# nloyfer/wgbs_tools

Measured on AMD Instinct MI355X. Metric: CpG-sites/sec segmented, higher is better.
Workload: dtype u8 counts -> u32 prefix sums -> f32/f64 log-likelihood (bit-exact with the reference)

## Files before the change

### wgbs_tools_amd/build.py

```python
import os
import os.path as op
import shutil
import subprocess
import sys

HERE = op.dirname(op.abspath(__file__))
CSRC = op.join(HERE, 'csrc')
ARCH = 'gfx950'
HIPFLAGS = ['--offload-arch=' + ARCH, '-O3', '-std=c++17', '-ffp-contract=off', '-fPIC', '-shared', '-pthread']

TARGETS = {
    'libwgbsseg.so': (['wgbsseg.hip'], ['owners.h', 'env.h', 'seg_kernels.h', 'block_plan.h', 'block_kernels.h', 'plain_dp.h', 'wave_prims.h', 'exact_log2.h', 'stitch.h', 'add_loci.h', 'table_io.h', 'pat_kernels.h', 'homog_kernels.h', 'bimodal_kernels.h', 'stats_kernels.h', 'pair_plan.h', 'pair_kernels.h', '../../include/wgbsseg.h']),
    'libwgbssynth.so': (['synth.hip'], []),
}


def source_hash():
    import hashlib
    srcs, hdrs = TARGETS['libwgbsseg.so']
    h = hashlib.sha256()
    for f in sorted(op.normpath(op.join(CSRC, x)) for x in srcs + hdrs):
        with open(f, 'rb') as fh:
            h.update(fh.read())
    return h.hexdigest()[:16]


def hipcc():
    for cand in (shutil.which('hipcc'), '/opt/rocm/bin/hipcc'):
        if cand and op.isfile(cand):
            return cand
    raise RuntimeError('hipcc not found: cannot build the gfx950 libraries')


PROGRAMS = {
    'segmentor': (['segmentor_main.cpp'], ['../../include/wgbsseg.h']),
# ... 40 lines not shown
```

### wgbs_tools_amd/csrc/seg_kernels.h

```cpp
#pragma once
#include <hip/hip_runtime.h>
#include <stddef.h>
#include <stdint.h>
#include "exact_log2.h"
#include "wave_prims.h"

#ifndef WG_CARRY_SHIFT
#define WG_CARRY_SHIFT  7
#endif
#define WG_SCAN_STAGED  512
#define WG_CARRY_G      (1 << WG_CARRY_SHIFT)
static_assert(WG_CARRY_SHIFT >= 4 && WG_CARRY_SHIFT <= 10, "k_scan: a lane vector is 16 sites, an iteration 1024");
#define WG_BLOCK        256
#define WG_WIN_TILE     1024
#define WG_PAIR_CAP     4096
#define WG_TRACE_WIN    32768
#define WG_NARROW_WMAX  60
#define WG_MEDIUM_WMAX  252
#define WG_MEDIUM_TS    16

__device__ const wg_log_tables g_wg_tables = WG_LOG_TABLES_INIT;

__device__ __forceinline__ void wg_fast_tables_to_lds(wg_fast_tables* ft, int tid, int nthreads)
{
    const double* f = reinterpret_cast<const double*>(g_wg_tables.f_tab);
    const double* d = reinterpret_cast<const double*>(g_wg_tables.d_tab);
    double* of = reinterpret_cast<double*>(ft->f_tab);
    double* od = reinterpret_cast<double*>(ft->d_fast);
// ... 636 lines not shown
            t[j] = in ? ((h >> 8) & 0xffu) : 0u;
            tot += m[j] | (t[j] << 16);
        }
        const uint32_t incl = wg_wave_incl_scan_dpp_u32(tot);
        const uint32_t excl = incl - tot;
        uint32_t em = run_m + (excl & 0xffffu), et = run_t + (excl >> 16);
#pragma unroll
        for (int j = 0; j < 4; j++) {
            const int x = sidx + j - hs;
            if (x >= x0 && x < cnt) dst[x - x0] = make_uint2(em, et);
            em += m[j]; et += t[j];
        }
        const uint32_t wt = (uint32_t)__builtin_amdgcn_readlane((int)incl, 63);
        run_m += wt & 0xffffu; run_t += wt >> 16;
    }
}

__device__ __forceinline__ int wg_group_start(const ChunkDesc& cd, int k)
{
    const int64_t a = (cd.start0 + k) & ~(int64_t)(WG_CARRY_G - 1);
    return a <= cd.start0 ? 0 : (int)(a - cd.start0);
}

template <int ROW>
__device__ __forceinline__ void wg_stage_local_rows(uint32_t* __restrict__ Et, const uint8_t* __restrict__ betas, int64_t pitch,
                                                    int s_first, int ns, const ChunkDesc& cd, int64_t n_total, int ka, int cnt,
                                                    int lane, int wv)
{
    constexpr bool WHOLE = ROW > 128;
    const int half = WHOLE ? 0 : lane >> 5, l5 = WHOLE ? lane : lane & 31;
    const int64_t abs0 = cd.start0 + ka;
    const int64_t al = abs0 & ~3LL;
    const int hs = (int)(abs0 - al);
    const int sidx = l5 * 4;
    const int64_t a = al + sidx;
    const int nsite = cnt - 1;
    for (int r0 = WHOLE ? wv : wv * 2; r0 < ns; r0 += (WHOLE ? 1 : 2) * (WG_BLOCK / 64)) {
        const int rr = r0 + half;
        const bool act = rr < ns;
        uint32_t w0 = 0, w1 = 0;
        if (act && sidx < nsite + hs) {
            const uint8_t* row = betas + (int64_t)(s_first + rr) * pitch;
            if (a + 4 <= n_total) {
                const uint2 v = *reinterpret_cast<const uint2*>(row + 2 * a);
                w0 = v.x; w1 = v.y;
            } else {
                for (int j = 0; j < 4; j++) if (a + j < n_total) {
                    const uint32_t h = (uint32_t)row[2 * (a + j)] | ((uint32_t)row[2 * (a + j) + 1] << 8);
                    if (j < 2) w0 |= h << (16 * j); else w1 |= h << (16 * (j - 2));
                }
            }
        }
        uint32_t mt[4];
        uint32_t tot = 0;
#pragma unroll
        for (int j = 0; j < 4; j++) {
            const uint32_t h = ((j < 2) ? w0 : w1) >> (16 * (j & 1));
            const int x = sidx + j - hs;
            const bool in = x >= 0 && x < nsite;
            mt[j] = in ? ((h & 0xffu) | ((h & 0xff00u) << 8)) : 0u;
            tot += mt[j];
        }
        const uint32_t incl = WHOLE ? wg_wave_incl_scan_dpp_u32(tot) : wg_half_incl_scan_dpp_u32(tot);
        uint32_t e = incl - tot;
        uint32_t* dst = Et + (size_t)rr * ROW;
#pragma unroll
        for (int j = 0; j < 4; j++) {
            const int x = sidx + j - hs;
            if (act && x >= 0 && x < cnt) dst[x] = e;
            e += mt[j];
        }
    }
}

template <int ROW>
__device__ __forceinline__ void wg_stage_local_rows_long(uint32_t* __restrict__ Et, const uint8_t* __restrict__ betas, int64_t pitch,
                                                     int s_first, int ns, const ChunkDesc& cd, int64_t n_total, int ka, int cnt,
                                                     int lane, int wv)
{
    const int64_t abs0 = cd.start0 + ka;
    const int64_t al = abs0 & ~3LL;
    const int hs = (int)(abs0 - al);
    const int nsite = cnt - 1;
    for (int rr = wv; rr < ns; rr += WG_BLOCK / 64) {
        const uint8_t* row = betas + (int64_t)(s_first + rr) * pitch;
        uint32_t* dst = Et + (size_t)rr * ROW;
        uint32_t run = 0;
        for (int p0 = 0; p0 < nsite + hs; p0 += 256) {
            const int sidx = p0 + lane * 4;
            const int64_t a = al + sidx;
            uint32_t w0 = 0, w1 = 0;
            if (sidx < nsite + hs) {
                if (a + 4 <= n_total) {
                    const uint2 v = *reinterpret_cast<const uint2*>(row + 2 * a);
// ... 7 lines not shown
            }
            uint32_t mt[4];
            uint32_t tot = 0;
#pragma unroll
            for (int j = 0; j < 4; j++) {
                const uint32_t h = ((j < 2) ? w0 : w1) >> (16 * (j & 1));
                const int x = sidx + j - hs;
                const bool in = x >= 0 && x < nsite;
                mt[j] = in ? ((h & 0xffu) | ((h & 0xff00u) << 8)) : 0u;
                tot += mt[j];
            }
            const uint32_t incl = wg_wave_incl_scan_dpp_u32(tot);
            uint32_t e = run + (incl - tot);
#pragma unroll
            for (int j = 0; j < 4; j++) {
                const int x = sidx + j - hs;
                if (x >= 0 && x < cnt) dst[x] = e;
                e += mt[j];
            }
            run += (uint32_t)__builtin_amdgcn_readlane((int)incl, 63);
        }
        if (lane == 0 && ((nsite + hs) & 255) == 0 && nsite < cnt) dst[nsite] = run;
    }
}

#define WG_WIDE_TK      128
#define WG_WIDE_TS      16

template <int TI, int FAST, int SPLIT, bool ONEG>
__global__ __launch_bounds__(WG_BLOCK) void k_cost(JobView J, StageView SV, CostArgs A, const TileDesc* __restrict__ tiles,
                                                   int64_t n_tiles, double* __restrict__ cost, int64_t n_tiles_padded)
{
    constexpr bool WIDE = SPLIT == 1;
    constexpr int WM = SPLIT == 2 ? WG_MEDIUM_WMAX : WG_NARROW_WMAX;
    static_assert(SPLIT != 2 || TI == WG_MEDIUM_TS, "a medium tile is one 16-site unit");
    constexpr int KS = WIDE ? WG_WIDE_TK + 1 : TI + WM + 1;
    constexpr int IS = WIDE ? WG_WIDE_TS + 1 : 0;
    constexpr bool KY = (FAST >= 2);
    constexpr bool DIVS = (FAST == 3);
    extern __shared__ __attribute__((aligned(16))) char smem[];
    static_assert(sizeof(wg_fast_tables) % 16 == 0 && sizeof(wg_d2) == 16, "the arrays behind the tables are 16-byte aligned");
    const size_t TB = KY ? (size_t)A.rows * (16 + 64) * sizeof(wg_d2) : sizeof(wg_fast_tables);
    wg_fast_tables* tb = reinterpret_cast<wg_fast_tables*>(smem);
    wg_d2* iyt = reinterpret_cast<wg_d2*>(smem);
    wg_d2* kyt = iyt + (size_t)A.rows * 16;
    const wg_d2* iy0 = iyt + (A.rows - 1) * 16;
    const wg_d2* ky0 = kyt + (A.rows - 1) * 64;
    uint2* Et = reinterpret_cast<uint2*>(smem + TB);
    uint2* St = Et + (size_t)A.NS * KS;
    uint32_t* Lt = reinterpret_cast<uint32_t*>(smem + TB);
    char* after = WIDE ? reinterpret_cast<char*>(St + (((size_t)A.NS * (KS + IS) + 1) & ~(size_t)1) - (size_t)A.NS * KS)
                       : reinterpret_cast<char*>(Lt + (((size_t)A.NS * KS + 3) & ~(size_t)3));
    struct Rec { int32_t offs, ea; int64_t sb; };
    Rec* rec = reinterpret_cast<Rec*>(after);
    int32_t* misc = reinterpret_cast<int32_t*>(rec + (TI + 1));
    uint8_t* cmap = reinterpret_cast<uint8_t*>(misc + 8);
    constexpr bool CMAP = !WIDE;

    const int tid = threadIdx.x, lane = tid & 63, wv = tid >> 6;
    const int nC = J.n_chunks;
    const int64_t G = A.xcd_group, jx = (int64_t)(blockIdx.x >> 3);
    const int64_t t = (jx / G) * (8 * G) + (int64_t)(blockIdx.x & 7) * G + (jx % G);
    if (t >= n_tiles) return;
    const TileDesc td = tiles[t];
    const int c = td.chunk;
    const ChunkDesc cd = J.chunks[c];
    const int ka = td.ka, nk = td.nk, kb = ka + nk;
    const int et_lo = WIDE ? td.et_lo : 0;
    const int et_hi = WIDE ? et_lo + WG_WIDE_TK : (1 << 30);
    const uint32_t cum0 = SV.cum0[(int64_t)SV.stage * nC + c];

    if (KY) wg_lookup_tables_to_lds(iyt, kyt, A.rows, A.tab, tid, WG_BLOCK);
    else wg_fast_tables_to_lds(tb, tid, WG_BLOCK);
    constexpr int PW = (TI + 63) / 64;
    if (wv < PW) {
        const int kl = wv * 64 + lane;
        const int k = ka + kl;
        const bool valid = kl < nk;
        int cnt = 0, is = 0, ie = -1;
        if (valid) {
            const int f = J.W16[cd.site_off + k];
            is = k > et_lo ? k : et_lo;
            ie = (k + f < et_hi ? k + f : et_hi) - 1;
            cnt = ie - is + 1;
            if (cnt < 0) cnt = 0;
// ... 68 lines not shown
            else while (hi - lo > 1) { const int mid = (lo + hi) >> 1; if (rec[mid].offs <= q) lo = mid; else hi = mid; }
            const Rec r = rec[lo];
            double acc = firstg ? 0.0 : accR[qi];
            auto term = [&](float nm, float nt) -> double {
                const float ll = FAST == 1 ? wg_sample_term(nm, nt, pc, pc2, tb, &g_wg_tables) : wg_sample_term_plain(nm, nt, pc, pc2, &g_wg_tables);
                return (double)ll;
            };
            if (WIDE) {
                const uint2* Ep = Et + (q + r.ea);
                const uint2* Sp = St + lo;
                auto one = [&](int sl) {
                    const uint2 pi = Ep[sl * KS];
                    const uint2 pk = Sp[sl * IS];
                    if (KY) acc += (double)wg_sample_term_pcpos_ks<DIVS>((float)(pi.x - pk.x), (float)(pi.y - pk.y), pc, pc2, iy0, ky0, &g_wg_tables);
                    else acc += term((float)(pi.x - pk.x), (float)(pi.y - pk.y));
                };
                int sl = 0;
                for (; sl + 4 <= ns; sl += 4) { one(sl); one(sl + 1); one(sl + 2); one(sl + 3); }
                for (; sl < ns; sl++) one(sl);
            } else {
                const uint32_t* Ep = Lt + (q + r.ea);
                const uint32_t* Sp = Lt + lo;
                auto one = [&](int sl) {
                    const uint32_t d = Ep[sl * KS] - Sp[sl * KS];
                    if (KY) acc += (double)wg_sample_term_pcpos_ks<DIVS>((float)(d & 0xffffu), (float)(d >> 16), pc, pc2, iy0, ky0, &g_wg_tables);
                    else acc += term((float)(d & 0xffffu), (float)(d >> 16));
                };
                int sl = 0;
                for (; sl + 4 <= ns; sl += 4) { one(sl); one(sl + 1); one(sl + 2); one(sl + 3); }
                for (; sl < ns; sl++) one(sl);
            }
            if (lastg) cb[r.sb + q] = acc;
            else accR[qi] = acc;
        }
    }
    if (A.finished != nullptr && tid == 0) __hip_atomic_fetch_add(A.finished, 1u, __ATOMIC_RELAXED, __HIP_MEMORY_SCOPE_AGENT);
}

#ifdef WGBSSEG_DP_TIMING
#define WG_DP_T(...) __VA_ARGS__
#else
#define WG_DP_T(...)
#endif
struct DpArgs { int32_t ringN; int32_t pad[3]; };

#define WG_DP_STATE_HDR 257

__device__ __forceinline__ double wg_ld_l2_f64(const double* p) { return __hip_atomic_load(p, __ATOMIC_RELAXED, __HIP_MEMORY_SCOPE_AGENT); }
__device__ __forceinline__ int32_t wg_ld_l2_i32(const int32_t* p) { return __hip_atomic_load(p, __ATOMIC_RELAXED, __HIP_MEMORY_SCOPE_AGENT); }

template <int NW, int BL>
struct DpRows {
    static constexpr int PER = (BL + NW - 1) / NW;
    double va[PER], vb[PER];
    uint32_t fmax;
    bool wideb;
};

struct DpMeta { uint32_t w, rel; };
// ... 993 lines not shown
```

### wgbs_tools_amd/csrc/wgbsseg.hip

```cpp
#include <hip/hip_runtime.h>
#include <algorithm>
#include <atomic>
#include <chrono>
#include <cstdarg>
#include <cstdio>
#include <cstdlib>
#include <cstring>
#include <deque>
#include <functional>
#include <initializer_list>
#include <memory>
#include <string>
#include <thread>
#include <vector>
#include <pthread.h>
#include <sched.h>
#include <sys/mman.h>
#if defined(__x86_64__) && !defined(__HIP_DEVICE_COMPILE__)
#include <emmintrin.h>
#endif

#include "../../include/wgbsseg.h"
#include "owners.h"
#include "seg_kernels.h"
// ... 82 lines not shown
    bool counted_live = false;
    double stage_gate_wide_evals = 100000.0, stage_min_evals_per_step = 21000.0;
    bool stage_gate_shared = false;
    int stage_gate = 768, last_stage_pct = -1, force_dp_mode = 0, force_ns = 0, force_ti = 0;
    double last_block_sums_ms = 0.0;
    int64_t table_blocks = 0;
    bool accumulate = false;
    std::vector<std::pair<int64_t, int64_t>> validated;
    DevBuf scan_pieces, divcheck, plan_sb;
    DevBuf bs_plan, bs_desc, bs_out;
    DevBuf mk_out, cv_in, cv_out;
    DevBuf st_ranges, st_parts;
    DevBuf ph_pairs, ph_edges, ph_out;
    std::vector<int32_t> h_stage_bounds;
    float divs_pc = -1.0f;
    bool divs_ok = false;
    int64_t last_dp_chunks = 0, last_dp_stride = 0;
    float divs_m_pc = -1.0f;
    bool divs_m_ok = false;
    bool divs_enabled = true, bs_general = false;
    int64_t scan_piece_sites = 4096;
    int medium_wmax = WG_MEDIUM_WMAX;
    bool dp_wlean = true, early = true, speculate = true, batch_marks = false;
    ~wgbsseg_ctx() { (void)hipSetDevice(device); (void)hipDeviceSynchronize(); }
};

namespace {

bool device_local_cpus(int device, NearCpus* out)
{
    out->valid = false;
    if (!env_flag("WGBSSEG_UPLOAD_PIN", true)) return false;
    char bus[64] = {0};
    if (hipDeviceGetPCIBusId(bus, (int)sizeof bus, device) != hipSuccess) { (void)hipGetLastError(); return false; }
    for (char* q = bus; *q; q++) if (*q >= 'A' && *q <= 'F') *q = (char)(*q - 'A' + 'a');
    char path[160];
    snprintf(path, sizeof path, "/sys/bus/pci/devices/%s/local_cpulist", bus);
    FILE* f = fopen(path, "r");
    if (!f) return false;
    char line[8192] = {0};
    const bool got = fgets(line, (int)sizeof line, f) != nullptr;
    fclose(f);
    if (!got) return false;
    const size_t bytes = CPU_ALLOC_SIZE(WG_MAX_CPUS);
    std::vector<unsigned long> allowed(bytes / sizeof(unsigned long), 0ul);
    out->bits.assign(bytes / sizeof(unsigned long), 0ul);
// ... 224 lines not shown
    HIP_TRY(c->evD.create(false));
    HIP_TRY(c->evS.create(false));
    for (auto& v : c->ev) HIP_TRY(v.create());
    const long long budget_mb = env_int("WGBSSEG_COST_BUDGET_MB", 0);
    c->cost_budget_bytes = (budget_mb > 0 ? budget_mb : 6144LL) << 20;
    c->force_stages = (int)env_int("WGBSSEG_FORCE_STAGES", 0);
    c->stage_gate = (int)env_int("WGBSSEG_STAGE_GATE", c->stage_gate, 0);
    c->stage_gate_shared = env_flag("WGBSSEG_STAGE_GATE_SHARED", false);
    c->stage_gate_wide_evals = env_double("WGBSSEG_STAGE_GATE_WIDE_EVALS", c->stage_gate_wide_evals);
    c->stage_min_evals_per_step = env_double("WGBSSEG_STAGE_MIN_EVALS", c->stage_min_evals_per_step);
    if (env_int("WGBSSEG_LAST_STAGE_PCT", -1) != -1) c->last_stage_pct = (int)env_int("WGBSSEG_LAST_STAGE_PCT", -1, 5, 800);
    c->force_dp_mode = (int)env_int("WGBSSEG_DP_MODE", 0, 0, 2);
    c->force_ns = (int)env_int("WGBSSEG_NS", 0);
    c->force_ti = (int)env_int("WGBSSEG_TI", 0);
    c->bs_general = env_flag("WGBSSEG_BLOCK_SUMS_GENERAL", false);
    c->divs_enabled = env_flag("WGBSSEG_DIV_SHORT", true);
    { const long long sp = env_int("WGBSSEG_SCAN_PIECE_SITES", 0); if (sp >= 1024) c->scan_piece_sites = sp & ~1023LL; }
    const int wm = (int)env_int("WGBSSEG_MEDIUM_WMAX", WG_MEDIUM_WMAX, 0, WG_MEDIUM_WMAX);
    c->medium_wmax = wm > WG_NARROW_WMAX ? wm : 0;
    c->dp_wlean = env_flag("WGBSSEG_DP_WLEAN", true);
    c->early = !env_flag("WGBSSEG_NO_EARLY", false);
    c->speculate = !env_flag("WGBSSEG_NO_SPECULATION", false);
    c->batch_marks = env_int("WGBSSEG_PROFILE", 0) >= 2;
    g_live_ctx[device & 63].fetch_add(1, std::memory_order_relaxed);
    c->counted_live = true;
    *out = c.release();
    return WGBSSEG_OK;
}
}
extern "C" {

int wgbsseg_create(int device, wgbsseg_ctx** out, char* err, size_t errlen) { return create_ctx(device, true, out, err, errlen); }

void wgbsseg_destroy(wgbsseg_ctx* c)
{
    if (!c) return;
    if (c->counted_live) g_live_ctx[c->device & 63].fetch_sub(1, std::memory_order_relaxed);
    const double t0 = wall_s();
    delete c;
    if (profiling()) fprintf(stderr, "[wgbsseg] destroy: %.1f ms\n", (wall_s() - t0) * 1e3);
}

static hipError_t own_rows(wgbsseg_ctx* c, int64_t n_samples, int64_t n_sites, int elem)
{
    const int64_t pitch = round_up(2 * elem * n_sites, 256) + 256;
    const hipError_t e = c->betas_own.ensure((size_t)pitch * (size_t)n_samples);
// ... 205 lines not shown
    return WGBSSEG_OK;
}

int launch_scan(wgbsseg_ctx* c, const Job& job, hipStream_t s, char* err, size_t errlen)
{
    const int64_t rows = (int64_t)job.v.n_chunks * job.v.n_samples;
    const int64_t blocks = (rows + (WG_BLOCK / 64) - 1) / (WG_BLOCK / 64);
    if (blocks > 0x7fffffff) { set_err(err, errlen, "too many (chunk, sample) rows"); return WGBSSEG_E_ARG; }
    hipLaunchKernelGGL(k_scan, dim3((unsigned)blocks), dim3(WG_BLOCK), 0, s, job.v, c->status.as<JobStatus>());
    HIP_TRY(hipGetLastError());
    return WGBSSEG_OK;
}

int report_bad_site(const wgbsseg_ctx* c, const JobStatus& st, char* err, size_t errlen)
{
    const long long s = (long long)(st.first_bad >> 40), site = (long long)(st.first_bad & ((1ULL << 40) - 1));
    uint8_t mc[2] = {0, 0};
    (void)hipMemcpy(mc, c->betas + s * c->pitch + 2 * site, 2, hipMemcpyDeviceToHost);
    set_err(err, errlen, "invalid data: sample %lld (0-based, argument order), site %lld (0-based): meth %d > cov %d",
            s, site + (long long)c->site_base, (int)mc[0], (int)mc[1]);
    return WGBSSEG_E_METH_GT_COV;
}

template <int TI, int FAST, int SPLIT>
hipError_t launch_cost(const JobView& v, const StageView& sv, const CostArgs& a, const TileDesc* td, int64_t tiles, double* cost, size_t lds, hipStream_t s)
{
    const int64_t padded = round_up(tiles, 8 * (int64_t)a.xcd_group);
    if (TI > 64 || a.NS >= v.n_samples)
        hipLaunchKernelGGL((k_cost<TI, FAST, SPLIT, true>), dim3((unsigned)padded), dim3(WG_BLOCK), lds, s, v, sv, a, td, tiles, cost, padded);
    else
        hipLaunchKernelGGL((k_cost<(TI > 64 ? 64 : TI), FAST, SPLIT, false>), dim3((unsigned)padded), dim3(WG_BLOCK), lds, s, v, sv, a, td, tiles, cost, padded);
    return hipGetLastError();
}

template <int FAST>
hipError_t launch_cost_fast(int cls, int TI, const JobView& v, const StageView& sv, const CostArgs& a, const TileDesc* td, int64_t tiles, double* cost, size_t lds, hipStream_t s)
{
    if (cls == 2) return launch_cost<WG_MEDIUM_TS, FAST, 2>(v, sv, a, td, tiles, cost, lds, s);
    if (cls == 1) return launch_cost<WG_WIDE_TS, FAST == 3 ? 2 : FAST, 1>(v, sv, a, td, tiles, cost, lds, s);
    if (TI == 128) return launch_cost<128, FAST, 0>(v, sv, a, td, tiles, cost, lds, s);
    if (TI == 64) return launch_cost<64, FAST, 0>(v, sv, a, td, tiles, cost, lds, s);
    if (TI == 32) return launch_cost<32, FAST, 0>(v, sv, a, td, tiles, cost, lds, s);
    return launch_cost<16, FAST, 0>(v, sv, a, td, tiles, cost, lds, s);
}
hipError_t launch_cost_class(int cls, int fast, int TI, const JobView& v, const StageView& sv, const CostArgs& a, const TileDesc* td, int64_t tiles, double* cost, size_t lds, hipStream_t s)
{
    return fast == 3 ? launch_cost_fast<3>(cls, TI, v, sv, a, td, tiles, cost, lds, s) : fast == 2 ? launch_cost_fast<2>(cls, TI, v, sv, a, td, tiles, cost, lds, s)
         : fast == 1 ? launch_cost_fast<1>(cls, TI, v, sv, a, td, tiles, cost, lds, s) : launch_cost_fast<0>(cls, TI, v, sv, a, td, tiles, cost, lds, s);
}

template <int FAST>
hipError_t set_cost_attrs()
{
    const void* fns[] = {reinterpret_cast<const void*>(&k_cost<128, FAST, 0, true>),
                         reinterpret_cast<const void*>(&k_cost<64, FAST, 0, true>), reinterpret_cast<const void*>(&k_cost<32, FAST, 0, true>),
                         reinterpret_cast<const void*>(&k_cost<16, FAST, 0, true>), reinterpret_cast<const void*>(&k_cost<WG_WIDE_TS, FAST == 3 ? 2 : FAST, 1, true>),
                         reinterpret_cast<const void*>(&k_cost<WG_MEDIUM_TS, FAST, 2, true>),
                         reinterpret_cast<const void*>(&k_cost<64, FAST, 0, false>), reinterpret_cast<const void*>(&k_cost<32, FAST, 0, false>),
                         reinterpret_cast<const void*>(&k_cost<16, FAST, 0, false>), reinterpret_cast<const void*>(&k_cost<WG_WIDE_TS, FAST == 3 ? 2 : FAST, 1, false>),
                         reinterpret_cast<const void*>(&k_cost<WG_MEDIUM_TS, FAST, 2, false>)};
    for (const void* f : fns) {
        const hipError_t e = hipFuncSetAttribute(f, hipFuncAttributeMaxDynamicSharedMemorySize, 160 * 1024);
        if (e != hipSuccess) return e;
    }
    return hipSuccess;
}
hipError_t set_kernel_attributes()
{
    hipError_t e = set_cost_attrs<0>();
    if (e == hipSuccess) e = set_cost_attrs<1>();
    if (e == hipSuccess) e = set_cost_attrs<2>();
    if (e == hipSuccess) e = set_cost_attrs<3>();
    const void* dps[] = {reinterpret_cast<const void*>(&k_dp<7, 64>), reinterpret_cast<const void*>(&k_dp<7, 64, true>),
                         reinterpret_cast<const void*>(&k_dp<7, 32>),
                         reinterpret_cast<const void*>(&k_dp<15, 32>)};
    for (const void* f : dps)
        if (e == hipSuccess) e = hipFuncSetAttribute(f, hipFuncAttributeMaxDynamicSharedMemorySize, 160 * 1024);
    return e;
}

void grow_events(std::vector<Event>& v, size_t n)
{
    while (v.size() < n) { v.emplace_back(); (void)v.back().create(); }
// ... 392 lines not shown
        if (hf[(size_t)i]) total += (int64_t)plain[(size_t)i].size();
        else { total += ooff[oi + 1] - ooff[oi]; oi++; }
    }
    borders_off[n_chunks] = total;
    int32_t* out = (*alloc)(total);
    if (!out) { set_err(err, errlen, "borders_out too small: need %lld ints", (long long)total); return WGBSSEG_E_CAPACITY; }
    oi = 0;
    for (int64_t i = 0; i < n_chunks; i++) {
        if (hf[(size_t)i]) memcpy(out + borders_off[i], plain[(size_t)i].data(), plain[(size_t)i].size() * 4);
        else { memcpy(out + borders_off[i], ob.data() + ooff[oi], (size_t)(ooff[oi + 1] - ooff[oi]) * 4); oi++; }
    }
    c->last_valid = false;
    return WGBSSEG_OK;
}

int Batch::tile_plan(char* err, size_t errlen)
{
    BatchPlan& p = plan;
    const float pc = P.pseudo_count;
    const int n_stages = p.n_stages;
    CostArgs base;
    memset(&base, 0, sizeof(base));
    base.pc = pc; base.pc2 = pc + pc;
    base.xcd_group = 64;
    base.cmap = 3;
    for (int k = 0; k < 3; k++) { ca[k] = base; ca[k].NS = p.NS[k]; ca[k].rows = p.rows[k]; }
    if (p.term_mode[0] == 2) {
        const bool same = c->lookup_pc == pc && c->lookup_rows[0] == p.rows[0] && c->lookup_rows[1] == p.rows[1] && c->lookup_rows[2] == p.rows[2] && c->lookup.p;
        if (!same) {
            static const wg_log_tables host_tabs = WG_LOG_TABLES_INIT;
            c->h_lookup.resize((size_t)(p.rows[0] + p.rows[1] + p.rows[2]) * 80);
            wg_d2* dst = c->h_lookup.data();
            for (int rows : p.rows) {
                for (int x = 0; x < rows * 16; x++) dst[x] = wg_ks_iy_entry(&host_tabs, rows, x);
                for (int x = 0; x < rows * 64; x++) dst[rows * 16 + x] = wg_ks_ky_entry(&host_tabs, rows, x);
                dst += (size_t)rows * 80;
            }
            HIP_TRY(c->lookup.ensure(c->h_lookup.size() * sizeof(wg_d2)));
            HIP_TRY(hipMemcpyAsync(c->lookup.p, c->h_lookup.data(), c->h_lookup.size() * sizeof(wg_d2), hipMemcpyHostToDevice, c->sA));
            c->lookup_pc = pc;
            for (int k = 0; k < 3; k++) c->lookup_rows[k] = p.rows[k];
        }
        const wg_d2* tab = c->lookup.as<wg_d2>();
        for (int k = 0; k < 3; k++) { ca[k].tab = tab; tab += (size_t)p.rows[k] * 80; }
    }
    const size_t sb_bytes = (size_t)(n_stages + 1) * 4;
    HIP_TRY(c->plan_sb.ensure(sb_bytes));
// ... 67 lines not shown
    HIP_TRY(c->tmp_borders.ensure((size_t)(job.sites_padded + nC) * 4));
    HIP_TRY(c->nb.ensure((size_t)nC * 4));
    out_head = (size_t)round_up((int64_t)(nC + 1) * 8, 16);
    c->out_par ^= 1;
    outb = &c->out_borders[c->out_par];
    HIP_TRY(outb->ensure(out_head + (size_t)(J + nC) * 4));
    for (auto* evs : {&c->ev_cost0, &c->ev_cost1, &c->ev_dp0, &c->ev_dp1, &c->ev_fork, &c->ev_join}) grow_events(*evs, n_stages);
    StageView sv;
    sv.cbase = c->plan_cbase.as<int64_t>(); sv.cum0 = c->plan_cum0.as<uint32_t>();
    sv.tbaseA = c->plan_tbase.as<int64_t>(); sv.tbaseB = sv.tbaseA + (size_t)n_stages * (nC + 1);
    sv.sb = c->plan_sb.as<int32_t>();
    DpArgs da = {p.ringN, {c->dp_wlean ? 0 : 1, 0, 0}};
#ifdef WGBSSEG_DP_TIMING
    da.pad[1] = (int)env_int("WGBSSEG_DP_DEBUG", 0);
#endif
    c->last_dp_chunks = nC; c->last_dp_stride = p.state_stride;
    const size_t lds_dp = 2 * 4096 * 8 + 128 * 8 + 64 * 12 + 16 + 1024 * 6;
    double* const dps = c->dpstate.as<double>();
    if (st.wide_units) HIP_TRY(hipStreamWaitEvent(c->sA, c->ev[EV_SCAN_END], 0));
    if (st.wide_units && p.gated) HIP_TRY(hipStreamWaitEvent(c->sA2, c->ev[EV_SCAN_END], 0));
    const bool divsA = c->divs_enabled && c->divs_ok && c->divs_pc == P.pseudo_count;
    const bool divsM = c->divs_enabled && c->divs_m_ok && c->divs_m_pc == P.pseudo_count;
    const int fast[3] = {p.term_mode[0] == 2 && divsA ? 3 : p.term_mode[0], p.term_mode[1], p.term_mode[2] == 2 && divsM ? 3 : p.term_mode[2]};
    for (int stg = 0; stg < n_stages; stg++) {
        const int64_t* const nt = &p.stage_tiles[3 * (size_t)stg];
        hipStream_t const sP = p.gated && (stg & 1) ? c->sA2 : c->sA;
        sv.stage = stg;
        double* cbuf = c->cost[stg % p.nbuf].as<double>();
        const bool side = nt[0] > 0 && (nt[1] > 0 || nt[2] > 0);
        hipStream_t const sSide = side ? (p.gated && (stg & 1) ? c->sA : c->sA2) : sP;
        if (stg >= p.nbuf) HIP_TRY(hipStreamWaitEvent(sP, c->ev_dp1[stg - p.nbuf], 0));
        if (p.gated) {
            const int64_t before = stg > 0 ? nt[-3] + nt[-2] + nt[-1] : 0;
            if (before > 0) {
                const double est_s = 10.0 * (double)p.stage_pairs[(size_t)stg - 1] * c->n_samples / 5e11;
                const long long max_ticks = (long long)(1e8 * std::min(2.0, std::max(0.005, est_s)));
                hipLaunchKernelGGL(k_stage_gate, dim3(1), dim3(64), 0, sP, (const uint32_t*)(c->stage_ctr.as<uint32_t>() + (stg - 1)),
                                   (uint32_t)std::max<int64_t>(1, before - c->stage_gate), max_ticks);
                HIP_TRY(hipGetLastError());
            }
            for (CostArgs& a : ca) a.finished = c->stage_ctr.as<uint32_t>() + stg;
        }
        HIP_TRY(hipEventRecord(c->ev_cost0[stg], sP));
        if (side) { HIP_TRY(hipEventRecord(c->ev_fork[stg], sP)); HIP_TRY(hipStreamWaitEvent(sSide, c->ev_fork[stg], 0)); }
        for (int k : {0, 2, 1})
            if (nt[k] > 0)
                HIP_TRY(launch_cost_class(k, fast[k], p.TI, v, sv, ca[k], c->tiles[k].as<TileDesc>() + tile0[k][(size_t)stg], nt[k], cbuf, p.lds[k], k == 0 ? sP : sSide));
        if (side) { HIP_TRY(hipEventRecord(c->ev_join[stg], sSide)); HIP_TRY(hipStreamWaitEvent(sP, c->ev_join[stg], 0)); }
        HIP_TRY(hipEventRecord(c->ev_cost1[stg], sP));
        HIP_TRY(hipStreamWaitEvent(c->sB, c->ev_cost1[stg], 0));
        HIP_TRY(hipEventRecord(c->ev_dp0[stg], c->sB));
        const bool dp16 = p.dp_mode == 0 && n_stages > 1 && stg + 1 < n_stages;
        if (dp16)                                  hipLaunchKernelGGL((k_dp16<3>), dim3((unsigned)nC), dim3(64 * 4), (size_t)(2 * 16 * 64 * 8 + WG_DP_META_RING * 6), c->sB, v, sv, cbuf, dps, p.state_stride);
        else if (p.dp_mode == 0 && p.all_narrow)   hipLaunchKernelGGL((k_dp<7, 64, true>), dim3((unsigned)nC), dim3(64 * 8), lds_dp, c->sB, v, sv, cbuf, da, dps, p.state_stride);
        else if (p.dp_mode == 0)                   hipLaunchKernelGGL((k_dp<7, 64>), dim3((unsigned)nC), dim3(64 * 8), lds_dp, c->sB, v, sv, cbuf, da, dps, p.state_stride);
        else if (p.dp_mode == 1)                   hipLaunchKernelGGL((k_dp<7, 32>), dim3((unsigned)nC), dim3(64 * 8), lds_dp, c->sB, v, sv, cbuf, da, dps, p.state_stride);
        else                                       hipLaunchKernelGGL((k_dp<15, 32>), dim3((unsigned)nC), dim3(64 * 16), lds_dp, c->sB, v, sv, cbuf, da, dps, p.state_stride);
        HIP_TRY(hipGetLastError());
        HIP_TRY(hipEventRecord(c->ev_dp1[stg], c->sB));
    }
    return WGBSSEG_OK;
}

int Batch::deliver(char* err, size_t errlen)
{
    int64_t* const d_boff = outb->as<int64_t>();
    int32_t* const d_bord = reinterpret_cast<int32_t*>(reinterpret_cast<char*>(outb->p) + out_head);
    HIP_TRY(hipEventRecord(c->ev[EV_TRACE0], c->sB));
    hipLaunchKernelGGL(k_trace, dim3((unsigned)nC), dim3(WG_BLOCK), 0, c->sB, job.v, c->tmp_borders.as<int32_t>(), c->nb.as<int32_t>());
    HIP_TRY(hipGetLastError());
// ... 1730 lines not shown
        set_err(err, errlen, "test_bimodal: the EM of block %llu (row of the blocks) did not settle within %d iterations", s->em_cap, WG_BIM_MAX_ITERS);
        return WGBSSEG_E_CAPACITY;
    }
    HIP_TRY(hipMemcpy(ll, b->res_f.p, (size_t)b->n_blocks * 24, hipMemcpyDeviceToHost));
    HIP_TRY(hipMemcpy(counts, b->res_i.p, (size_t)b->n_blocks * 24, hipMemcpyDeviceToHost));
    return WGBSSEG_OK;
}

double wgbsseg_bimodal_kernel_ms(wgbsseg_bimodal* b)
{
    return b ? b->feed.kernel_ms() : -1.0;
}

int wgbsseg_get_timings(const wgbsseg_ctx* c, wgbsseg_timings* out)
{
    if (!c || !out) return WGBSSEG_E_ARG;
    *out = c->tim;
    return WGBSSEG_OK;
}

int64_t wgbsseg_debug_fetch(wgbsseg_ctx* c, const char* what, void* out, int64_t cap_bytes)
{
    if (!c || !what || !out || !c->last_valid) return WGBSSEG_E_STATE;
    const void* src = nullptr;
    int64_t bytes = 0;
    if (!strcmp(what, "window")) { src = c->W16.p; bytes = c->last_sites * 2; }
    else if (!strcmp(what, "cum")) { src = c->cum32.p; bytes = c->last_sites * 4; }
    else if (!strcmp(what, "back")) { src = c->back16.p; bytes = c->last_sites * 2; }
    else if (!strcmp(what, "dpstate")) { src = c->dpstate.p; bytes = c->last_dp_chunks * c->last_dp_stride * 8; }
    else if (!strcmp(what, "cost")) { if (c->last_stages != 1) return WGBSSEG_E_STATE; src = c->cost[0].p; bytes = c->last_pairs * 8; }
    else return WGBSSEG_E_ARG;
    if (bytes > cap_bytes) return WGBSSEG_E_CAPACITY;
    if (hipSetDevice(c->device) != hipSuccess) return WGBSSEG_E_HIP;
    if (hipMemcpy(out, src, (size_t)bytes, hipMemcpyDeviceToHost) != hipSuccess) return WGBSSEG_E_HIP;
    return bytes;
}

int wgbsseg_debug_sample_terms(wgbsseg_ctx* c, const float* nmeth, const float* ntotal, int64_t count, float pseudo_count, float* out)
{
    char* err = nullptr; size_t errlen = 0;
    if (!c || !nmeth || !ntotal || !out || count < 1) return WGBSSEG_E_ARG;
    HIP_TRY(hipSetDevice(c->device));
    HIP_TRY(c->dbg_a.ensure((size_t)count * 4)); HIP_TRY(c->dbg_b.ensure((size_t)count * 4)); HIP_TRY(c->dbg_c.ensure((size_t)count * 4));
    HIP_TRY(hipMemcpyAsync(c->dbg_a.p, nmeth, (size_t)count * 4, hipMemcpyHostToDevice, c->sA));
    HIP_TRY(hipMemcpyAsync(c->dbg_b.p, ntotal, (size_t)count * 4, hipMemcpyHostToDevice, c->sA));
    const unsigned blocks = (unsigned)std::min<int64_t>((count + 255) / 256, 8192);
// ... 84 lines not shown
```

Baseline: 1.142 billion.

## Pair two narrow cost tiles per workgroup and prefetch the next tile's rows

Adds a k_cost_pair kernel in which each workgroup scores two consecutive narrow cost tiles (TI 64 or 128) from the same XCD group. While the first tile's term evaluation proceeds, the window, cum and first beta row words of the second tile are fetched into registers, to hide global load latency and amortise the LDS table staging across two tiles. It is enabled by default for ungated TI=64 narrow runs and selected through an env knob, with the row load and scan logic factored into shared helpers. The cost is higher register pressure from the prefetched fronts and half as many workgroups in flight.

Result: faster. 1.158 billion, median of 4 (+1.3%).

```diff
diff --git a/wgbs_tools_amd/build.py b/wgbs_tools_amd/build.py
--- a/wgbs_tools_amd/build.py
+++ b/wgbs_tools_amd/build.py
@@ -10,7 +10,7 @@
 HIPFLAGS = ['--offload-arch=' + ARCH, '-O3', '-std=c++17', '-ffp-contract=off', '-fPIC', '-shared', '-pthread']
 
 TARGETS = {
-    'libwgbsseg.so': (['wgbsseg.hip'], ['owners.h', 'env.h', 'seg_kernels.h', 'block_plan.h', 'block_kernels.h', 'plain_dp.h', 'wave_prims.h', 'exact_log2.h', 'stitch.h', 'add_loci.h', 'table_io.h', 'pat_kernels.h', 'homog_kernels.h', 'bimodal_kernels.h', 'stats_kernels.h', 'pair_plan.h', 'pair_kernels.h', '../../include/wgbsseg.h']),
+    'libwgbsseg.so': (['wgbsseg.hip'], ['owners.h', 'env.h', 'seg_kernels.h', 'cost_map.h', 'block_plan.h', 'block_kernels.h', 'plain_dp.h', 'wave_prims.h', 'exact_log2.h', 'stitch.h', 'add_loci.h', 'table_io.h', 'pat_kernels.h', 'homog_kernels.h', 'bimodal_kernels.h', 'stats_kernels.h', 'pair_plan.h', 'pair_kernels.h', '../../include/wgbsseg.h']),
     'libwgbssynth.so': (['synth.hip'], []),
 }
 
diff --git a/wgbs_tools_amd/csrc/cost_map.h b/wgbs_tools_amd/csrc/cost_map.h
--- /dev/null
+++ b/wgbs_tools_amd/csrc/cost_map.h
@@ -0,0 +1,15 @@
+#pragma once
+#include <stdint.h>
+#include "exact_log2.h"
+
+WG_HD int64_t wg_cost_tile(int64_t wg, int h, int per, int64_t G)
+{
+    const int64_t j = (wg >> 3) * per + h;
+    return (j / G) * (8 * G) + (wg & 7) * G + (j % G);
+}
+
+WG_HD int64_t wg_cost_grid(int64_t n_tiles, int per, int64_t G)
+{
+    const int64_t padded = (n_tiles + 8 * G - 1) / (8 * G) * (8 * G);
+    return ((padded + per - 1) / per + 7) / 8 * 8;
+}
diff --git a/wgbs_tools_amd/csrc/seg_kernels.h b/wgbs_tools_amd/csrc/seg_kernels.h
--- a/wgbs_tools_amd/csrc/seg_kernels.h
+++ b/wgbs_tools_amd/csrc/seg_kernels.h
@@ -4,6 +4,7 @@
 #include <stdint.h>
 #include "exact_log2.h"
 #include "wave_prims.h"
+#include "cost_map.h"
 
 #ifndef WG_CARRY_SHIFT
 #define WG_CARRY_SHIFT  7
@@ -686,6 +687,44 @@
     return a <= cd.start0 ? 0 : (int)(a - cd.start0);
 }
 
+__device__ __forceinline__ uint2 wg_local_row_words(const uint8_t* __restrict__ row, int64_t a, int64_t n_total, bool want)
+{
+    uint32_t w0 = 0, w1 = 0;
+    if (want) {
+        if (a + 4 <= n_total) {
+            const uint2 v = *reinterpret_cast<const uint2*>(row + 2 * a);
+            w0 = v.x; w1 = v.y;
+        } else {
+            for (int j = 0; j < 4; j++) if (a + j < n_total) {
+                const uint32_t h = (uint32_t)row[2 * (a + j)] | ((uint32_t)row[2 * (a + j) + 1] << 8);
+                if (j < 2) w0 |= h << (16 * j); else w1 |= h << (16 * (j - 2));
+            }
+        }
+    }
+    return make_uint2(w0, w1);
+}
+template <bool WHOLE>
+__device__ __forceinline__ void wg_local_row_scan(uint32_t* __restrict__ dst, const uint2 w, bool act, int sidx, int hs, int nsite, int cnt)
+{
+    uint32_t mt[4];
+    uint32_t tot = 0;
+#pragma unroll
+    for (int j = 0; j < 4; j++) {
+        const uint32_t h = ((j < 2) ? w.x : w.y) >> (16 * (j & 1));
+        const int x = sidx + j - hs;
+        const bool in = x >= 0 && x < nsite;
+        mt[j] = in ? ((h & 0xffu) | ((h & 0xff00u) << 8)) : 0u;
+        tot += mt[j];
+    }
+    const uint32_t incl = WHOLE ? wg_wave_incl_scan_dpp_u32(tot) : wg_half_incl_scan_dpp_u32(tot);
+    uint32_t e = incl - tot;
+#pragma unroll
+    for (int j = 0; j < 4; j++) {
+        const int x = sidx + j - hs;
+        if (act && x >= 0 && x < cnt) dst[x] = e;
+        e += mt[j];
+    }
+}
 template <int ROW>
 __device__ __forceinline__ void wg_stage_local_rows(uint32_t* __restrict__ Et, const uint8_t* __restrict__ betas, int64_t pitch,
                                                     int s_first, int ns, const ChunkDesc& cd, int64_t n_total, int ka, int cnt,
@@ -702,38 +741,8 @@
     for (int r0 = WHOLE ? wv : wv * 2; r0 < ns; r0 += (WHOLE ? 1 : 2) * (WG_BLOCK / 64)) {
         const int rr = r0 + half;
         const bool act = rr < ns;
-        uint32_t w0 = 0, w1 = 0;
-        if (act && sidx < nsite + hs) {
-            const uint8_t* row = betas + (int64_t)(s_first + rr) * pitch;
-            if (a + 4 <= n_total) {
-                const uint2 v = *reinterpret_cast<const uint2*>(row + 2 * a);
-                w0 = v.x; w1 = v.y;
-            } else {
-                for (int j = 0; j < 4; j++) if (a + j < n_total) {
-                    const uint32_t h = (uint32_t)row[2 * (a + j)] | ((uint32_t)row[2 * (a + j) + 1] << 8);
-                    if (j < 2) w0 |= h << (16 * j); else w1 |= h << (16 * (j - 2));
-                }
-            }
-        }
-        uint32_t mt[4];
-        uint32_t tot = 0;
-#pragma unroll
-        for (int j = 0; j < 4; j++) {
-            const uint32_t h = ((j < 2) ? w0 : w1) >> (16 * (j & 1));
-            const int x = sidx + j - hs;
-            const bool in = x >= 0 && x < nsite;
-            mt[j] = in ? ((h & 0xffu) | ((h & 0xff00u) << 8)) : 0u;
-            tot += mt[j];
-        }
-        const uint32_t incl = WHOLE ? wg_wave_incl_scan_dpp_u32(tot) : wg_half_incl_scan_dpp_u32(tot);
-        uint32_t e = incl - tot;
-        uint32_t* dst = Et + (size_t)rr * ROW;
-#pragma unroll
-        for (int j = 0; j < 4; j++) {
-            const int x = sidx + j - hs;
-            if (act && x >= 0 && x < cnt) dst[x] = e;
-            e += mt[j];
-        }
+        const uint2 w = wg_local_row_words(betas + (int64_t)(s_first + rr) * pitch, a, n_total, act && sidx < nsite + hs);
+        wg_local_row_scan<WHOLE>(Et + (size_t)rr * ROW, w, act, sidx, hs, nsite, cnt);
     }
 }
 
@@ -787,6 +796,14 @@
         }
         if (lane == 0 && ((nsite + hs) & 255) == 0 && nsite < cnt) dst[nsite] = run;
     }
+}
+
+template <int FAST>
+__device__ __forceinline__ double wg_packed_term(uint32_t d, float pc, float pc2, const wg_fast_tables* tb, const wg_d2* iy0, const wg_d2* ky0)
+{
+    const float nm = (float)(d & 0xffffu), nt = (float)(d >> 16);
+    if (FAST >= 2) return (double)wg_sample_term_pcpos_ks<FAST == 3>(nm, nt, pc, pc2, iy0, ky0, &g_wg_tables);
+    return (double)(FAST == 1 ? wg_sample_term(nm, nt, pc, pc2, tb, &g_wg_tables) : wg_sample_term_plain(nm, nt, pc, pc2, &g_wg_tables));
 }
 
 #define WG_WIDE_TK      128
@@ -824,8 +841,7 @@
 
     const int tid = threadIdx.x, lane = tid & 63, wv = tid >> 6;
     const int nC = J.n_chunks;
-    const int64_t G = A.xcd_group, jx = (int64_t)(blockIdx.x >> 3);
-    const int64_t t = (jx / G) * (8 * G) + (int64_t)(blockIdx.x & 7) * G + (jx % G);
+    const int64_t t = wg_cost_tile((int64_t)blockIdx.x, 0, 1, A.xcd_group);
     if (t >= n_tiles) return;
     const TileDesc td = tiles[t];
     const int c = td.chunk;
@@ -940,9 +956,7 @@
                 const uint32_t* Ep = Lt + (q + r.ea);
                 const uint32_t* Sp = Lt + lo;
                 auto one = [&](int sl) {
-                    const uint32_t d = Ep[sl * KS] - Sp[sl * KS];
-                    if (KY) acc += (double)wg_sample_term_pcpos_ks<DIVS>((float)(d & 0xffffu), (float)(d >> 16), pc, pc2, iy0, ky0, &g_wg_tables);
-                    else acc += term((float)(d & 0xffffu), (float)(d >> 16));
+                    acc += wg_packed_term<FAST>(Ep[sl * KS] - Sp[sl * KS], pc, pc2, tb, iy0, ky0);
                 };
                 int sl = 0;
                 for (; sl + 4 <= ns; sl += 4) { one(sl); one(sl + 1); one(sl + 2); one(sl + 3); }
@@ -953,6 +967,157 @@
         }
     }
     if (A.finished != nullptr && tid == 0) __hip_atomic_fetch_add(A.finished, 1u, __ATOMIC_RELAXED, __HIP_MEMORY_SCOPE_AGENT);
+}
+
+template <int TI, int FAST>
+__global__ __launch_bounds__(WG_BLOCK) void k_cost_pair(JobView J, StageView SV, CostArgs A, const TileDesc* __restrict__ tiles, int64_t n_tiles,
+                                                        double* __restrict__ cost)
+{
+    static_assert(TI == 64 || TI == 128, "paired tiles: the 64- and 128-start narrow tiles");
+    constexpr int WM = WG_NARROW_WMAX, KS = TI + WM + 1;
+    constexpr bool KY = (FAST >= 2), WHOLE = KS > 128;
+    constexpr int PW = (TI + 63) / 64;
+    constexpr int RPP = (WHOLE ? 1 : 2) * (WG_BLOCK / 64);
+    constexpr int NPRE = 4;
+    extern __shared__ __attribute__((aligned(16))) char smem[];
+    const size_t TB = KY ? (size_t)A.rows * (16 + 64) * sizeof(wg_d2) : sizeof(wg_fast_tables);
+    wg_fast_tables* tb = reinterpret_cast<wg_fast_tables*>(smem);
+    wg_d2* iyt = reinterpret_cast<wg_d2*>(smem);
+    wg_d2* kyt = iyt + (size_t)A.rows * 16;
+    const wg_d2* iy0 = iyt + (A.rows - 1) * 16;
+    const wg_d2* ky0 = kyt + (A.rows - 1) * 64;
+    uint32_t* Lt = reinterpret_cast<uint32_t*>(smem + TB);
+    struct Rec { int32_t offs, ea; int64_t sb; };
+    Rec* rec = reinterpret_cast<Rec*>(Lt + (((size_t)A.NS * KS + 3) & ~(size_t)3));
+    int32_t* misc = reinterpret_cast<int32_t*>(rec + (TI + 1));
+    uint8_t* cmap = reinterpret_cast<uint8_t*>(misc + 8);
+
+    const int tid = threadIdx.x, lane = tid & 63, wv = tid >> 6;
+    const int nC = J.n_chunks, ns = J.n_samples;
+    const int64_t t0 = wg_cost_tile((int64_t)blockIdx.x, 0, 2, A.xcd_group);
+    if (t0 >= n_tiles) return;
+    const int64_t t1 = wg_cost_tile((int64_t)blockIdx.x, 1, 2, A.xcd_group);
+    const int np = t1 < n_tiles ? 2 : 1;
+
+    if (KY) wg_lookup_tables_to_lds(iyt, kyt, A.rows, A.tab, tid, WG_BLOCK);
+    else wg_fast_tables_to_lds(tb, tid, WG_BLOCK);
+
+    const int half = WHOLE ? 0 : lane >> 5, sidx = (WHOLE ? lane : lane & 31) * 4;
+    struct Desc {
+        int32_t ka, nk;
+        uint32_t cum0;
+        int64_t start0, site_off;
+        int64_t cbase;
+    };
+    auto describe = [&](int64_t t) {
+        const TileDesc td = tiles[t];
+        const ChunkDesc* cd = J.chunks + td.chunk;
+        Desc D;
+        D.ka = td.ka; D.nk = td.nk; D.start0 = cd->start0; D.site_off = cd->site_off;
+        D.cum0 = SV.cum0[(int64_t)SV.stage * nC + td.chunk];
+        D.cbase = SV.cbase[(int64_t)SV.stage * nC + td.chunk];
+        return D;
+    };
+    struct Front {
+        int32_t f;
+        uint32_t cum;
+        uint2 w[NPRE];
+    };
+    auto fetch = [&](const Desc& D, Front& F) {
+        const int kl = wv * 64 + lane;
+        const bool valid = wv < PW && kl < D.nk;
+        F.f = valid ? (int)J.W16[D.site_off + D.ka + kl] : 0;
+        F.cum = valid ? J.cum32[D.site_off + D.ka + kl] : 0u;
+        const int64_t abs0 = D.start0 + D.ka, al = abs0 & ~3LL;
+        const bool inrow = sidx < D.nk + WM + (int)(abs0 - al);
+#pragma unroll
+        for (int p = 0; p < NPRE; p++) {
+            const int rr = (WHOLE ? wv : wv * 2) + p * RPP + half;
+            F.w[p] = wg_local_row_words(J.betas + (int64_t)rr * J.pitch, al + sidx, J.n_total, rr < ns && inrow);
+        }
+    };
+
+    const Desc D0 = describe(t0), D1 = describe(np > 1 ? t1 : t0);
+    const float pc = A.pc, pc2 = A.pc2;
+    auto score = [&](const Desc& D, const Front& F, bool more, const Desc& Dn, Front& N) {
+        const int ka = D.ka, nk = D.nk;
+        if (wv < PW) {
+            const int kl = wv * 64 + lane, k = ka + kl;
+            const bool valid = kl < nk;
+            const int cnt = F.f;
+            const uint32_t incl = wg_wave_incl_scan_dpp_u32((uint32_t)cnt);
+            if (kl < TI) {
+                const int32_t o = (int32_t)(incl - (uint32_t)cnt);
+                const int is = valid ? k : 0;
+                Rec r;
+                r.offs = o;
+                r.ea = is - o + 1 - ka;
+                r.sb = (valid ? (int64_t)(F.cum - D.cum0) - k : 0) + (is - o);
+                rec[kl] = r;
+            }
+            const uint32_t imax = wg_wave_max_u32(cnt > 0 ? (uint32_t)(k + cnt - 1) : 0u);
+            if (lane == 0) misc[2 * wv + 1] = (int32_t)imax;
+            if (lane == 63) misc[4 + wv] = (int32_t)incl;
+        }
+        __syncthreads();
+        const int imax = PW > 1 ? (misc[1] > misc[3] ? misc[1] : misc[3]) : misc[1];
+        const int Q = PW > 1 ? misc[4] + misc[5] : misc[4];
+        if (Q > 0) {
+            if (PW > 1) {
+                if (wv == 1 && lane < TI - 64) {
+                    const int q0 = misc[4];
+                    Rec& r = rec[64 + lane];
+                    r.offs += q0; r.sb -= q0; r.ea -= q0;
+                }
+                __syncthreads();
+            }
+            if (tid == 0) rec[nk].offs = Q;
+            if (tid < nk) {
+                const int o0 = rec[tid].offs, o1 = tid + 1 < nk ? rec[tid + 1].offs : Q;
+                const int sh = A.cmap;
+                for (int g = (o0 + (1 << sh) - 1) >> sh; (g << sh) < o1; g++) cmap[g] = (uint8_t)tid;
+            }
+            const int Ecnt = imax + 2 - ka, nsite = Ecnt - 1;
+            const int64_t abs0 = D.start0 + ka, al = abs0 & ~3LL;
+            const int hs = (int)(abs0 - al);
+#pragma unroll
+            for (int p = 0; p < NPRE; p++) {
+                const int r0 = (WHOLE ? wv : wv * 2) + p * RPP, rr = r0 + half;
+                if (r0 < ns) wg_local_row_scan<WHOLE>(Lt + (size_t)rr * KS, F.w[p], rr < ns, sidx, hs, nsite, Ecnt);
+            }
+            for (int r0 = (WHOLE ? wv : wv * 2) + NPRE * RPP; r0 < ns; r0 += RPP) {
+                const int rr = r0 + half;
+                const uint2 w = wg_local_row_words(J.betas + (int64_t)rr * J.pitch, al + sidx, J.n_total, rr < ns && sidx < nsite + hs);
+                wg_local_row_scan<WHOLE>(Lt + (size_t)rr * KS, w, rr < ns, sidx, hs, nsite, Ecnt);
+            }
+        }
+        if (more) fetch(Dn, N);
+        if (Q > 0) {
+            __syncthreads();
+            double* cb = cost + D.cbase;
+            for (int q = tid; q < Q; q += WG_BLOCK) {
+                int lo = (int)cmap[q >> A.cmap];
+                if (A.cmap) while (rec[lo + 1].offs <= q) lo++;
+                const Rec r = rec[lo];
+                double acc = 0.0;
+                const uint32_t* Ep = Lt + (q + r.ea);
+                const uint32_t* Sp = Lt + lo;
+                auto one = [&](int sl) { acc += wg_packed_term<FAST>(Ep[sl * KS] - Sp[sl * KS], pc, pc2, tb, iy0, ky0); };
+                int sl = 0;
+                for (; sl + 4 <= ns; sl += 4) { one(sl); one(sl + 1); one(sl + 2); one(sl + 3); }
+                for (; sl < ns; sl++) one(sl);
+                cb[r.sb + q] = acc;
+            }
+        }
+    };
+    Front F0, F1;
+    fetch(D0, F0);
+    score(D0, F0, np > 1, D1, F1);
+    if (np > 1) {
+        __syncthreads();
+        score(D1, F1, false, D1, F0);
+    }
+    if (A.finished != nullptr && tid == 0) __hip_atomic_fetch_add(A.finished, (uint32_t)np, __ATOMIC_RELAXED, __HIP_MEMORY_SCOPE_AGENT);
 }
 
 #ifdef WGBSSEG_DP_TIMING
diff --git a/wgbs_tools_amd/csrc/wgbsseg.hip b/wgbs_tools_amd/csrc/wgbsseg.hip
--- a/wgbs_tools_amd/csrc/wgbsseg.hip
+++ b/wgbs_tools_amd/csrc/wgbsseg.hip
@@ -128,6 +128,8 @@
     int64_t scan_piece_sites = 4096;
     int medium_wmax = WG_MEDIUM_WMAX;
     bool dp_wlean = true, early = true, speculate = true, batch_marks = false;
+    int cost_pair = 1;
+    int32_t last_cost_forms[2] = {0, 0};
     ~wgbsseg_ctx() { (void)hipSetDevice(device); (void)hipDeviceSynchronize(); }
 };
 
@@ -398,6 +400,7 @@
     c->early = !env_flag("WGBSSEG_NO_EARLY", false);
     c->speculate = !env_flag("WGBSSEG_NO_SPECULATION", false);
     c->batch_marks = env_int("WGBSSEG_PROFILE", 0) >= 2;
+    c->cost_pair = (int)env_int("WGBSSEG_COST_PAIR", c->cost_pair, 0, 2);
     g_live_ctx[device & 63].fetch_add(1, std::memory_order_relaxed);
     c->counted_live = true;
     *out = c.release();
@@ -649,10 +652,19 @@
     return WGBSSEG_E_METH_GT_COV;
 }
 
+constexpr int WG_XCD_GROUP = 64;
+static_assert(WG_XCD_GROUP % 2 == 0, "paired tiles: both slots of a workgroup in one XCD group");
+
 template <int TI, int FAST, int SPLIT>
-hipError_t launch_cost(const JobView& v, const StageView& sv, const CostArgs& a, const TileDesc* td, int64_t tiles, double* cost, size_t lds, hipStream_t s)
-{
-    const int64_t padded = round_up(tiles, 8 * (int64_t)a.xcd_group);
+hipError_t launch_cost(const JobView& v, const StageView& sv, const CostArgs& a, const TileDesc* td, int64_t tiles, double* cost, size_t lds, hipStream_t s, bool pair)
+{
+    const int64_t padded = wg_cost_grid(tiles, 1, a.xcd_group);
+    if constexpr (SPLIT == 0 && (TI == 64 || TI == 128)) {
+        if (pair && a.NS >= v.n_samples && a.xcd_group % 2 == 0) {
+            hipLaunchKernelGGL((k_cost_pair<TI, FAST>), dim3((unsigned)wg_cost_grid(tiles, 2, a.xcd_group)), dim3(WG_BLOCK), lds, s, v, sv, a, td, tiles, cost);
+            return hipGetLastError();
+        }
+    }
     if (TI > 64 || a.NS >= v.n_samples)
         hipLaunchKernelGGL((k_cost<TI, FAST, SPLIT, true>), dim3((unsigned)padded), dim3(WG_BLOCK), lds, s, v, sv, a, td, tiles, cost, padded);
     else
@@ -661,19 +673,19 @@
 }
 
 template <int FAST>
-hipError_t launch_cost_fast(int cls, int TI, const JobView& v, const StageView& sv, const CostArgs& a, const TileDesc* td, int64_t tiles, double* cost, size_t lds, hipStream_t s)
-{
-    if (cls == 2) return launch_cost<WG_MEDIUM_TS, FAST, 2>(v, sv, a, td, tiles, cost, lds, s);
-    if (cls == 1) return launch_cost<WG_WIDE_TS, FAST == 3 ? 2 : FAST, 1>(v, sv, a, td, tiles, cost, lds, s);
-    if (TI == 128) return launch_cost<128, FAST, 0>(v, sv, a, td, tiles, cost, lds, s);
-    if (TI == 64) return launch_cost<64, FAST, 0>(v, sv, a, td, tiles, cost, lds, s);
-    if (TI == 32) return launch_cost<32, FAST, 0>(v, sv, a, td, tiles, cost, lds, s);
-    return launch_cost<16, FAST, 0>(v, sv, a, td, tiles, cost, lds, s);
-}
-hipError_t launch_cost_class(int cls, int fast, int TI, const JobView& v, const StageView& sv, const CostArgs& a, const TileDesc* td, int64_t tiles, double* cost, size_t lds, hipStream_t s)
-{
-    return fast == 3 ? launch_cost_fast<3>(cls, TI, v, sv, a, td, tiles, cost, lds, s) : fast == 2 ? launch_cost_fast<2>(cls, TI, v, sv, a, td, tiles, cost, lds, s)
-         : fast == 1 ? launch_cost_fast<1>(cls, TI, v, sv, a, td, tiles, cost, lds, s) : launch_cost_fast<0>(cls, TI, v, sv, a, td, tiles, cost, lds, s);
+hipError_t launch_cost_fast(int cls, int TI, const JobView& v, const StageView& sv, const CostArgs& a, const TileDesc* td, int64_t tiles, double* cost, size_t lds, hipStream_t s, bool pair)
+{
+    if (cls == 2) return launch_cost<WG_MEDIUM_TS, FAST, 2>(v, sv, a, td, tiles, cost, lds, s, false);
+    if (cls == 1) return launch_cost<WG_WIDE_TS, FAST == 3 ? 2 : FAST, 1>(v, sv, a, td, tiles, cost, lds, s, false);
+    if (TI == 128) return launch_cost<128, FAST, 0>(v, sv, a, td, tiles, cost, lds, s, pair);
+    if (TI == 64) return launch_cost<64, FAST, 0>(v, sv, a, td, tiles, cost, lds, s, pair);
+    if (TI == 32) return launch_cost<32, FAST, 0>(v, sv, a, td, tiles, cost, lds, s, false);
+    return launch_cost<16, FAST, 0>(v, sv, a, td, tiles, cost, lds, s, false);
+}
+hipError_t launch_cost_class(int cls, int fast, int TI, const JobView& v, const StageView& sv, const CostArgs& a, const TileDesc* td, int64_t tiles, double* cost, size_t lds, hipStream_t s, bool pair)
+{
+    return fast == 3 ? launch_cost_fast<3>(cls, TI, v, sv, a, td, tiles, cost, lds, s, pair) : fast == 2 ? launch_cost_fast<2>(cls, TI, v, sv, a, td, tiles, cost, lds, s, pair)
+         : fast == 1 ? launch_cost_fast<1>(cls, TI, v, sv, a, td, tiles, cost, lds, s, pair) : launch_cost_fast<0>(cls, TI, v, sv, a, td, tiles, cost, lds, s, pair);
 }
 
 template <int FAST>
@@ -685,7 +697,8 @@
                          reinterpret_cast<const void*>(&k_cost<WG_MEDIUM_TS, FAST, 2, true>),
                          reinterpret_cast<const void*>(&k_cost<64, FAST, 0, false>), reinterpret_cast<const void*>(&k_cost<32, FAST, 0, false>),
                          reinterpret_cast<const void*>(&k_cost<16, FAST, 0, false>), reinterpret_cast<const void*>(&k_cost<WG_WIDE_TS, FAST == 3 ? 2 : FAST, 1, false>),
-                         reinterpret_cast<const void*>(&k_cost<WG_MEDIUM_TS, FAST, 2, false>)};
+                         reinterpret_cast<const void*>(&k_cost<WG_MEDIUM_TS, FAST, 2, false>),
+                         reinterpret_cast<const void*>(&k_cost_pair<128, FAST>), reinterpret_cast<const void*>(&k_cost_pair<64, FAST>)};
     for (const void* f : fns) {
         const hipError_t e = hipFuncSetAttribute(f, hipFuncAttributeMaxDynamicSharedMemorySize, 160 * 1024);
         if (e != hipSuccess) return e;
@@ -1124,7 +1137,7 @@
     CostArgs base;
     memset(&base, 0, sizeof(base));
     base.pc = pc; base.pc2 = pc + pc;
-    base.xcd_group = 64;
+    base.xcd_group = WG_XCD_GROUP;
     base.cmap = 3;
     for (int k = 0; k < 3; k++) { ca[k] = base; ca[k].NS = p.NS[k]; ca[k].rows = p.rows[k]; }
     if (p.term_mode[0] == 2) {
@@ -1238,6 +1251,9 @@
     const bool divsA = c->divs_enabled && c->divs_ok && c->divs_pc == P.pseudo_count;
     const bool divsM = c->divs_enabled && c->divs_m_ok && c->divs_m_pc == P.pseudo_count;
     const int fast[3] = {p.term_mode[0] == 2 && divsA ? 3 : p.term_mode[0], p.term_mode[1], p.term_mode[2] == 2 && divsM ? 3 : p.term_mode[2]};
+    const bool pair = p.all_narrow && c->cost_pair >= (p.gated || p.TI != 64 ? 2 : 1);
+    const bool pair_form = pair && ca[0].NS >= v.n_samples && (p.TI == 64 || p.TI == 128);
+    c->last_cost_forms[0] = c->last_cost_forms[1] = 0;
     for (int stg = 0; stg < n_stages; stg++) {
         const int64_t* const nt = &p.stage_tiles[3 * (size_t)stg];
         hipStream_t const sP = p.gated && (stg & 1) ? c->sA2 : c->sA;
@@ -1261,7 +1277,8 @@
         if (side) { HIP_TRY(hipEventRecord(c->ev_fork[stg], sP)); HIP_TRY(hipStreamWaitEvent(sSide, c->ev_fork[stg], 0)); }
         for (int k : {0, 2, 1})
             if (nt[k] > 0)
-                HIP_TRY(launch_cost_class(k, fast[k], p.TI, v, sv, ca[k], c->tiles[k].as<TileDesc>() + tile0[k][(size_t)stg], nt[k], cbuf, p.lds[k], k == 0 ? sP : sSide));
+                HIP_TRY(launch_cost_class(k, fast[k], p.TI, v, sv, ca[k], c->tiles[k].as<TileDesc>() + tile0[k][(size_t)stg], nt[k], cbuf, p.lds[k], k == 0 ? sP : sSide, pair));
+        if (nt[0] > 0) c->last_cost_forms[pair_form ? 1 : 0]++;
         if (side) { HIP_TRY(hipEventRecord(c->ev_join[stg], sSide)); HIP_TRY(hipStreamWaitEvent(sP, c->ev_join[stg], 0)); }
         HIP_TRY(hipEventRecord(c->ev_cost1[stg], sP));
         HIP_TRY(hipStreamWaitEvent(c->sB, c->ev_cost1[stg], 0));
@@ -3038,6 +3055,11 @@
 int64_t wgbsseg_debug_fetch(wgbsseg_ctx* c, const char* what, void* out, int64_t cap_bytes)
 {
     if (!c || !what || !out || !c->last_valid) return WGBSSEG_E_STATE;
+    if (!strcmp(what, "cost_forms")) {
+        if (cap_bytes < (int64_t)sizeof c->last_cost_forms) return WGBSSEG_E_CAPACITY;
+        memcpy(out, c->last_cost_forms, sizeof c->last_cost_forms);
+        return (int64_t)sizeof c->last_cost_forms;
+    }
     const void* src = nullptr;
     int64_t bytes = 0;
     if (!strcmp(what, "window")) { src = c->W16.p; bytes = c->last_sites * 2; }
```
